# Snowdar/asv-subtools

Hardware: AMD Instinct MI355X
Metric: utterances/sec (200-frame) embedding extraction + EER, 1/2/4/8 MI355X (higher is better)
Workload: dtype bf16; 1 GPU; BASELINE configs[1]: standard TDNN x-vector: Xvector(80,10,training=False), 80-dim fbank, 256 utterances x 200 frames per GPU per step, features resident in HBM, f32 embeddings out; global_batch_utts=256, frames_per_utt=200, parallelism=utterance shards x1, streams=2

## Files before the change

### asv-subtools_amd/csrc/device_utils.h

```cpp
#pragma once
#include <hip/hip_runtime.h>
#include <stdint.h>

#include "asv_internal.h"

namespace asv {

typedef __attribute__((__vector_size__(8 * sizeof(__bf16)))) __bf16 bf16x8_t;
typedef __attribute__((__vector_size__(16 * sizeof(float)))) float f32x16_t;
typedef __attribute__((__vector_size__(4 * sizeof(float)))) float f32x4_t;

__host__ __device__ __forceinline__ int round_up_dev(int x, int m) { return (x + m - 1) / m * m; }

typedef _Float16 f16x8_t __attribute__((ext_vector_type(8)));
typedef _Float16 asv_f16x2 __attribute__((ext_vector_type(2)));

__device__ __forceinline__ float bf16_bits_to_f32(uint32_t h) { return __uint_as_float(h << 16); }

typedef float asv_f32x2 __attribute__((ext_vector_type(2)));
typedef __bf16 asv_bf16x2 __attribute__((ext_vector_type(2)));

__device__ __forceinline__ uint32_t pack_bf16x2(float lo, float hi) {
  const asv_f32x2 v = {lo, hi};
  return __builtin_bit_cast(uint32_t, __builtin_convertvector(v, asv_bf16x2));
}

__device__ __forceinline__ uint32_t f32_to_bf16_bits(float f) { return pack_bf16x2(f, 0.0f) & 0xffffu; }

template <int ET>
__device__ __forceinline__ uint32_t pack_h16x2(float lo, float hi) {
  static_assert(ET == ET_BF16 || ET == ET_F16, "16-bit element types only");
  const asv_f32x2 v = {lo, hi};
  if constexpr (ET == ET_BF16) return __builtin_bit_cast(uint32_t, __builtin_convertvector(v, asv_bf16x2));
  else return __builtin_bit_cast(uint32_t, __builtin_convertvector(v, asv_f16x2));
}
template <int ET>
__device__ __forceinline__ void unpack_h16x2(uint32_t w, float &lo, float &hi) {
  static_assert(ET == ET_BF16 || ET == ET_F16, "16-bit element types only");
  if constexpr (ET == ET_BF16) {
    lo = __uint_as_float(w << 16);
    hi = __uint_as_float(w & 0xffff0000u);
  } else {
    const asv_f32x2 f = __builtin_convertvector(__builtin_bit_cast(asv_f16x2, w), asv_f32x2);
    lo = f.x; hi = f.y;
  }
}
template <int ET>
__device__ __forceinline__ float h16_bits_to_f32(uint32_t h) {
  float lo, hi;
  unpack_h16x2<ET>(h, lo, hi);
  return lo;
}
template <int ET>
__device__ __forceinline__ uint32_t f32_to_h16_bits(float f) { return pack_h16x2<ET>(f, 0.0f) & 0xffffu; }

template <int ET>
__device__ __forceinline__ void unpack_h16x8(const uint4 u, float *v) {
  unpack_h16x2<ET>(u.x, v[0], v[1]); unpack_h16x2<ET>(u.y, v[2], v[3]);
  unpack_h16x2<ET>(u.z, v[4], v[5]); unpack_h16x2<ET>(u.w, v[6], v[7]);
}
template <int ET>
__device__ __forceinline__ uint4 pack_h16x8(const float *v) {
  return make_uint4(pack_h16x2<ET>(v[0], v[1]), pack_h16x2<ET>(v[2], v[3]), pack_h16x2<ET>(v[4], v[5]), pack_h16x2<ET>(v[6], v[7]));
}

template <int ET>
__device__ __forceinline__ f32x16_t mfma16(const uint4 a, const uint4 b, const f32x16_t c) {
  static_assert(ET == ET_BF16 || ET == ET_F16, "16-bit element types only");
  if constexpr (ET == ET_BF16) return __builtin_amdgcn_mfma_f32_32x32x16_bf16(__builtin_bit_cast(bf16x8_t, a), __builtin_bit_cast(bf16x8_t, b), c, 0, 0, 0);
  else return __builtin_amdgcn_mfma_f32_32x32x16_f16(__builtin_bit_cast(f16x8_t, a), __builtin_bit_cast(f16x8_t, b), c, 0, 0, 0);
}

__device__ __forceinline__ uint32_t relu_h16x2(uint32_t w) {
  typedef short s16x2 __attribute__((ext_vector_type(2)));
  const s16x2 z = {0, 0};
  return __builtin_bit_cast(uint32_t, __builtin_elementwise_max(__builtin_bit_cast(s16x2, w), z));
}

template <int ET>
__device__ __forceinline__ uint4 add_h16x8(uint4 a, uint4 b) {
  float va[8], vb[8];
  unpack_h16x8<ET>(a, va);
  unpack_h16x8<ET>(b, vb);
#pragma unroll
  for (int i = 0; i < 8; ++i) va[i] += vb[i];
  return pack_h16x8<ET>(va);
}
__device__ __forceinline__ uint4 add_bf16x8(uint4 a, uint4 b) { return add_h16x8<ET_BF16>(a, b); }

__device__ __forceinline__ uint4 add_f32x4(uint4 a, uint4 b) {
  uint4 r;
  r.x = __float_as_uint(__uint_as_float(a.x) + __uint_as_float(b.x));
  r.y = __float_as_uint(__uint_as_float(a.y) + __uint_as_float(b.y));
  r.z = __float_as_uint(__uint_as_float(a.z) + __uint_as_float(b.z));
  r.w = __float_as_uint(__uint_as_float(a.w) + __uint_as_float(b.w));
  return r;
}

struct X3Frag { uint4 hi, lo; };

__device__ __forceinline__ uint32_t h16_range_bits(uint32_t packed_hi) { return (packed_hi & 0x7fff7fffu) + 0x04000400u; }
__device__ __forceinline__ void x3_publish_range(uint32_t acc_bits, uint32_t *status) {
  if (status != nullptr && __builtin_amdgcn_ballot_w64((acc_bits & 0x80008000u) != 0u) != 0ull && (threadIdx.x & 63) == 0) atomicOr(status, ASV_STATUS_HALF_RANGE);
}

template <int ET, bool WITH_LO>
__device__ __forceinline__ X3Frag x3_split(const uint4 a, const uint4 b) {
  const float v[8] = {__uint_as_float(a.x), __uint_as_float(a.y), __uint_as_float(a.z), __uint_as_float(a.w),
                      __uint_as_float(b.x), __uint_as_float(b.y), __uint_as_float(b.z), __uint_as_float(b.w)};
  uint32_t h[4], l[4];
#pragma unroll
  for (int k = 0; k < 4; ++k) {
    h[k] = pack_h16x2<ET>(v[2 * k], v[2 * k + 1]);
    l[k] = 0u;
    if constexpr (WITH_LO) {
      float r0, r1;
      if constexpr (ET == ET_F16) {
        asm("v_fma_mix_f32 %0, %1, -1.0, %2 op_sel:[0,0,0] op_sel_hi:[1,0,0]" : "=v"(r0) : "v"(h[k]), "v"(v[2 * k]));
        asm("v_fma_mix_f32 %0, %1, -1.0, %2 op_sel:[1,0,0] op_sel_hi:[1,0,0]" : "=v"(r1) : "v"(h[k]), "v"(v[2 * k + 1]));
      } else {
        float h0, h1;
        unpack_h16x2<ET>(h[k], h0, h1);
        r0 = v[2 * k] - h0; r1 = v[2 * k + 1] - h1;
      }
      l[k] = pack_h16x2<ET>(r0, r1);
    }
  }
  X3Frag f;
  f.hi = make_uint4(h[0], h[1], h[2], h[3]);
  f.lo = make_uint4(l[0], l[1], l[2], l[3]);
  return f;
}
template <int ET, bool WITH_LO>
__device__ __forceinline__ X3Frag x3_split(const uint4 a, const uint4 b, uint32_t &range) {
  const X3Frag f = x3_split<ET, WITH_LO>(a, b);
  if constexpr (ET == ET_F16) range |= h16_range_bits(f.hi.x) | h16_range_bits(f.hi.y) | h16_range_bits(f.hi.z) | h16_range_bits(f.hi.w);
  return f;
}

constexpr int kScaleWhi = 127 + 6, kScaleWlo = 127 - 6, kScaleXlo = 127 - 11, kScaleXhi = 127;
typedef int v8i __attribute__((ext_vector_type(8)));

__device__ __forceinline__ uint32_t mx_range_bits(uint32_t packed_hi) { return (packed_hi & 0x7fff7fffu) + 0x05000500u; }

template <bool SEL>
__device__ __forceinline__ void split_mx(float v0, float v1, uint32_t &hi16, int &hi8, int &lo8, uint32_t &range) {
  hi16 = pack_h16x2<ET_F16>(v0, v1);
  range |= mx_range_bits(hi16);
  float r0, r1;
  asm("v_fma_mix_f32 %0, %1, -1.0, %2 op_sel:[0,0,0] op_sel_hi:[1,0,0]" : "=v"(r0) : "v"(hi16), "v"(v0));
  asm("v_fma_mix_f32 %0, %1, -1.0, %2 op_sel:[1,0,0] op_sel_hi:[1,0,0]" : "=v"(r1) : "v"(hi16), "v"(v1));
  hi8 = __builtin_amdgcn_cvt_pk_bf8_f32(v0, v1, hi8, SEL);
  lo8 = __builtin_amdgcn_cvt_pk_bf8_f32(r0 * 2048.0f, r1 * 2048.0f, lo8, SEL);
}

__device__ __forceinline__ double wave_sum_f64(double v) {
#pragma unroll
  for (int off = 32; off >= 1; off >>= 1) v += __shfl_xor(v, off);
  return v;
}

struct TrNo { static constexpr bool value = false; };
struct TrYes { static constexpr bool value = true; };

__device__ __forceinline__ float max_lo(float v, float lo) {
  float r;
  asm("v_max_f32 %0, %1, %2" : "=v"(r) : "v"(v), "v"(lo));
  return r;
}

__device__ __forceinline__ float apply_act(float v, int act) {
  switch (act) {
    case ASV_ACT_RELU: return fmaxf(v, 0.0f);
    case ASV_ACT_TANH: return tanhf(v);
    case ASV_ACT_SIGMOID: return 1.0f / (1.0f + expf(-v));
    default: return v;
  }
}

template <int ET>
__device__ __forceinline__ float load_elem(const void *base, size_t idx) {
  if constexpr (ET != ET_F32) return h16_bits_to_f32<ET>(reinterpret_cast<const uint16_t *>(base)[idx]);
  else return reinterpret_cast<const float *>(base)[idx];
}

template <int ET>
__device__ __forceinline__ void store_elem(void *base, size_t idx, float v) {
  if constexpr (ET != ET_F32) reinterpret_cast<uint16_t *>(base)[idx] = (uint16_t)f32_to_h16_bits<ET>(v);
  else reinterpret_cast<float *>(base)[idx] = v;
}

template <int RES_ET>
__device__ __forceinline__ float tdnn_epilogue(const TdnnKernelParams &p, float acc, int row, int ch,
                                               float bias, float scale, float shift, bool valid) {
  if (!valid) return 0.0f;
  float z = acc + bias;
  int seg = 0;
  if (p.seg_bias != nullptr || p.seg_scale != nullptr) seg = p.row_seg[row];
  if (p.seg_bias != nullptr) z += p.seg_bias[(size_t)seg * p.ld_segbias + ch];
  if (p.affine_first) {
    z = apply_act(z * scale + shift, p.act1);
  } else {
    z = apply_act(z, p.act1) * scale + shift;
  }
  z = apply_act(z, p.act2);
  if (p.seg_scale != nullptr) z *= p.seg_scale[(size_t)seg * p.ld_segscale + ch];
  if (p.res != nullptr) z += load_elem<RES_ET>(p.res, (size_t)row * p.ldres + ch);
  return z;
}

__device__ __forceinline__ float tdnn_epilogue_fast(float acc, float bias, float lo, float scale, float shift, bool valid) {
  const float z = fmaxf(acc + bias, lo) * scale + shift;
  return valid ? z : 0.0f;
}

__device__ __forceinline__ int xcd_swizzle(int bid, int nblocks) {
  const int xcd = bid & 7, q = nblocks >> 3, r = nblocks & 7;
  const int base = (xcd < r) ? xcd * (q + 1) : r * (q + 1) + (xcd - r) * q;
  return base + (bid >> 3);
}

}
```

### asv-subtools_amd/csrc/kernels_tdnn_chain.hip

```cpp
#include <cstdlib>

#include "chain_pool.h"
#include "lds_dma.h"

#ifndef CHAIN_EXP
#define CHAIN_EXP 0
#endif

namespace asv {
namespace {

constexpr int CN = kChainWidth;
constexpr int CBK = 64;
constexpr int CROWB = 128;
constexpr int CSTAGES = 4;
constexpr int YROWB = CN * 2;
template <int MF> struct ChainGeom {
  static constexpr int CM = MF * 32;
  static constexpr int CWIN = CM + 2 * kHalo;
  static constexpr int CSTAGE = CWIN * CROWB;
  static constexpr int CGROUPS = CWIN / 8;
  static constexpr int CPIECES = (CGROUPS + 7) / 8;
  static constexpr int Y_BYTES = CM * YROWB;
  static constexpr int SCR_OFF = Y_BYTES;
  static constexpr int LDS = Y_BYTES + 32768;
  static_assert(CSTAGES * CSTAGE <= Y_BYTES, "the window ring lives inside the Y region");
  static_assert(LDS <= 163840, "160 KiB of LDS per CU");
};

typedef float f32x2_t __attribute__((ext_vector_type(2)));

template <int POOLV, int ET = ET_BF16, int ABL = 0, int MF = 4>
__global__ __launch_bounds__(512, 2) void tdnn_chain_kernel(const TdnnChainParams p) {
  using Geo = ChainGeom<MF>;
  constexpr int CM = Geo::CM, CSTAGE = Geo::CSTAGE, CGROUPS = Geo::CGROUPS, CPIECES = Geo::CPIECES, SCR_OFF = Geo::SCR_OFF;
  __shared__ __attribute__((aligned(16))) unsigned char lds[Geo::LDS];
  const int tid = threadIdx.x, lane = tid & 63;
  const int wave = __builtin_amdgcn_readfirstlane(tid >> 6);
  const int lr = lane & 31, lh = lane >> 5;
  const int m0 = p.row_base + blockIdx.x * CM;
  const uint32_t lds_base = __builtin_amdgcn_readfirstlane((uint32_t)(uintptr_t)(lds_byte *)lds);
  float *par = reinterpret_cast<float *>(lds + SCR_OFF);

  int n_stamp = 0;
  auto stamp = [&]() {
    if (p.dbg != nullptr && lane == 0 && n_stamp < 14) p.dbg[((size_t)blockIdx.x * 8 + wave) * 32 + n_stamp] = __builtin_amdgcn_s_memtime();
    ++n_stamp;
  };
  auto fine = [&](int k) {
    if constexpr (ABL == 3) if (p.dbg != nullptr && lane == 0) p.dbg[((size_t)blockIdx.x * 8 + wave) * 32 + 16 + k] = __builtin_amdgcn_s_memtime();
  };
  stamp();
  if (p.dbg != nullptr && lane == 0) p.dbg[((size_t)blockIdx.x * 8 + wave) * 32 + 14] = __builtin_amdgcn_s_memrealtime();
  auto stage_params = [&](const TdnnChainLayer &L) {
    if (tid < 384) {
      const int which = tid >> 7, idx = (tid & 127) * 4;
      float4 v = (which == 1) ? make_float4(1.f, 1.f, 1.f, 1.f) : make_float4(0.f, 0.f, 0.f, 0.f);
      const float *src = (which == 0) ? L.bias : (which == 1 ? L.scale : L.shift);
      if (src != nullptr) v = *reinterpret_cast<const float4 *>(src + idx);
      *reinterpret_cast<float4 *>(par + which * CN + idx) = v;
    }
  };

  uint4 wf[4][2];
  f32x16_t acc[MF][2];
  struct XFrags { uint4 x[MF]; };
  auto init_acc = [&](const float *bias64) {
#pragma unroll
    for (int j = 0; j < 2; ++j)
#pragma unroll
      for (int q = 0; q < 4; ++q) {
        const float4 b4 = *reinterpret_cast<const float4 *>(bias64 + j * 32 + 8 * q + 4 * lh);
#pragma unroll
        for (int i = 0; i < MF; ++i) {
          acc[i][j][q * 4 + 0] = b4.x; acc[i][j][q * 4 + 1] = b4.y; acc[i][j][q * 4 + 2] = b4.z; acc[i][j][q * 4 + 3] = b4.w;
        }
      }
  };
  auto mma2 = [&](const XFrags &f, int kg, int j, int i0, auto tr) {
#pragma unroll
    for (int i = i0; i < i0 + 2 && i < MF; ++i) {
      if constexpr (decltype(tr)::value) acc[i][j] = mfma16<ET>(f.x[i], wf[kg][j], acc[i][j]);
      else acc[i][j] = mfma16<ET>(wf[kg][j], f.x[i], acc[i][j]);
    }
  };

  stage_params(p.first);
  {
    const unsigned char *xg = reinterpret_cast<const unsigned char *>(p.x);
    const size_t x_pitch = (size_t)p.ldx * 2;
    const int g_row = lane >> 3, g_slot = lane & 7;
    const int nchunks = p.cin_pad / CBK;
    const int n_taps = p.n_taps;
    uint32_t a_off[CPIECES];
#pragma unroll
    for (int i = 0; i < CPIECES; ++i) {
      const int grp = min(wave + i * 8, CGROUPS - 1);
      const int w = grp * 8 + g_row;
      const int row = min(max(m0 - kHalo + w, 0), p.rows - 1);
      a_off[i] = (uint32_t)row * (uint32_t)x_pitch + (uint32_t)lds_swz(w, g_slot) * 16u;
    }
    auto issue_A = [&](int c, int st) {
      const unsigned char *base = xg + (size_t)c * (CBK * 2);
#pragma unroll
      for (int i = 0; i < CPIECES; ++i) {
        const int grp = min(wave + i * 8, CGROUPS - 1);
        const uint32_t dst = __builtin_amdgcn_readfirstlane(lds_base + st * CSTAGE + grp * 1024);
        glds16_s(base, a_off[i], dst);
      }
    };
    const size_t frag_stride = (size_t)n_taps * nchunks * 4096;
    const unsigned char *wA0 = reinterpret_cast<const unsigned char *>(p.first.wfrag) + (size_t)(wave * 2) * frag_stride;
    const unsigned char *wA1 = wA0 + frag_stride;
    const uint32_t lane16 = (uint32_t)lane * 16u;
    auto x_base = [&](int c, int d) -> uint32_t {
      const int wrow = lr + kHalo + d;
      return (uint32_t)((c % CSTAGES) * CSTAGE + wrow * CROWB + ((lh ^ ((wrow >> 1) & 7)) << 4));
    };
    auto load_x4 = [&](uint32_t xb, int kg, int i, XFrags &f) {
      f.x[i] = *reinterpret_cast<const uint4 *>(lds + (xb ^ (uint32_t)(kg << 5)) + i * 4096);
    };
    issue_A(0, 0);
#pragma unroll
    for (int kg = 0; kg < 4; ++kg) {
      wf[kg][0] = *reinterpret_cast<const uint4 *>(wA0 + (size_t)kg * 1024 + lane16);
      wf[kg][1] = *reinterpret_cast<const uint4 *>(wA1 + (size_t)kg * 1024 + lane16);
    }
    if (nchunks > 2) {
      issue_A(1, 1);
      issue_A(2, 2);
      asm volatile("s_waitcnt vmcnt(%0)" ::"n"(2 * CPIECES) : "memory");
    } else {
      if (nchunks > 1) issue_A(1, 1);
      asm volatile("s_waitcnt vmcnt(0)" ::: "memory");
    }
    __builtin_amdgcn_s_barrier();
    asm volatile("" ::: "memory");
    stamp();
    init_acc(p.first.bias + wave * 64);
    const int v_taps = p.taps[lane < 9 ? lane : 0];
    const int d_first = __builtin_amdgcn_readlane(v_taps, 0);
    XFrags x0, x1;
    uint32_t xb = x_base(0, d_first);
#pragma unroll
    for (int i = 0; i < MF; ++i) load_x4(xb, 0, i, x0);
#pragma unroll 1
    for (int c = 0; c < nchunks; ++c) {
      for (int t = 0; t < n_taps; ++t) {
        const bool last_tap = (t + 1 == n_taps);
        int cn = c, tn = t + 1;
        if (last_tap) { tn = 0; cn = c + 1; }
        const bool more = cn < nchunks;
        if (!more) { cn = c; tn = t; }
        const size_t wnext = ((size_t)tn * nchunks + cn) * 4096;
        auto group = [&](const XFrags &xc, int kg, XFrags &xn, uint32_t xbn, int kgn) {
#pragma unroll
          for (int q = 0; q < 4; ++q) {
            if (q < MF) load_x4(xbn, kgn, q, xn);
            mma2(xc, kg, q / 2, (q % 2) * 2, TrNo{});
            if (q == 1) wf[kg][0] = *reinterpret_cast<const uint4 *>(wA0 + wnext + (size_t)kg * 1024 + lane16);
            if (q == 3) wf[kg][1] = *reinterpret_cast<const uint4 *>(wA1 + wnext + (size_t)kg * 1024 + lane16);
            __builtin_amdgcn_sched_barrier(0);
          }
        };
        group(x0, 0, x1, xb, 1);
        group(x1, 1, x0, xb, 2);
        group(x0, 2, x1, xb, 3);
        if (last_tap && c + 1 < nchunks) {
          asm volatile("s_waitcnt vmcnt(8)" ::: "memory");
          __builtin_amdgcn_s_barrier();
          asm volatile("" ::: "memory");
          if (c + 3 < nchunks) issue_A(c + 3, (c + 3) % CSTAGES);
        }
        const uint32_t xbn = x_base(cn, __builtin_amdgcn_readlane(v_taps, tn));
        group(x1, 3, x0, xbn, 0);
        xb = xbn;
      }
    }
  }

  auto store_Y = [&](int relu, bool affine) {
    const float act_lo = relu ? 0.0f : -INFINITY;
    unsigned char *yrow = lds + lr * YROWB + lh * 8;
    const int rx = lr & 15;
    if (!affine) {
#pragma unroll
      for (int j = 0; j < 2; ++j)
#pragma unroll
        for (int q = 0; q < 4; ++q) {
          unsigned char *dst = yrow + (((wave * 8 + j * 4 + q) ^ rx) << 4);
#pragma unroll
          for (int i = 0; i < MF; ++i) {
            uint2 pk;
            pk.x = pack_h16x2<ET>(acc[i][j][q * 4 + 0], acc[i][j][q * 4 + 1]);
            pk.y = pack_h16x2<ET>(acc[i][j][q * 4 + 2], acc[i][j][q * 4 + 3]);
            if (relu) { pk.x = relu_h16x2(pk.x); pk.y = relu_h16x2(pk.y); }
            *reinterpret_cast<uint2 *>(dst + i * 32 * YROWB) = pk;
          }
        }
      return;
    }
#pragma unroll
    for (int j = 0; j < 2; ++j)
#pragma unroll
      for (int q = 0; q < 4; ++q) {
        const int chl = wave * 64 + j * 32 + 8 * q + 4 * lh;
        const float4 sc4 = *reinterpret_cast<const float4 *>(par + CN + chl);
        const float4 sh4 = *reinterpret_cast<const float4 *>(par + 2 * CN + chl);
        const float sc[4] = {sc4.x, sc4.y, sc4.z, sc4.w}, sh[4] = {sh4.x, sh4.y, sh4.z, sh4.w};
        unsigned char *dst = yrow + (((wave * 8 + j * 4 + q) ^ rx) << 4);
#pragma unroll
        for (int i = 0; i < MF; ++i) {
          float y[4];
#pragma unroll
          for (int e = 0; e < 4; ++e) y[e] = fmaf(max_lo(acc[i][j][q * 4 + e], act_lo), sc[e], sh[e]);
          uint2 pk;
          pk.x = pack_h16x2<ET>(y[0], y[1]);
          pk.y = pack_h16x2<ET>(y[2], y[3]);
          *reinterpret_cast<uint2 *>(dst + i * 32 * YROWB) = pk;
        }
      }
  };

  auto yloop = [&](const unsigned char *wb0, const unsigned char *wb1, const float *bias64, auto tr) {
    const uint32_t lane16 = (uint32_t)lane * 16u;
    const uint32_t yb = (uint32_t)(lr * YROWB);
    const uint32_t sx = (uint32_t)(lh ^ (lr & 15));
    auto load_y4 = [&](int c, int kg, int i, XFrags &f) {
      f.x[i] = *reinterpret_cast<const uint4 *>(lds + yb + ((((uint32_t)(c * 8 + kg * 2)) ^ sx) << 4) + i * 32 * YROWB);
    };
#pragma unroll
    for (int kg = 0; kg < 4; ++kg) {
      wf[kg][0] = *reinterpret_cast<const uint4 *>(wb0 + (size_t)kg * 1024 + lane16);
      wf[kg][1] = *reinterpret_cast<const uint4 *>(wb1 + (size_t)kg * 1024 + lane16);
    }
    if constexpr (decltype(tr)::value) {
      const float b0 = bias64[lr], b1 = bias64[32 + lr];
#pragma unroll
      for (int i = 0; i < MF; ++i)
#pragma unroll
        for (int r = 0; r < 16; ++r) { acc[i][0][r] = b0; acc[i][1][r] = b1; }
    } else {
      init_acc(bias64);
    }
    XFrags x0, x1;
#pragma unroll
    for (int i = 0; i < MF; ++i) load_y4(0, 0, i, x0);
#pragma unroll 1
    for (int c = 0; c < CN / CBK; ++c) {
      const int cn = min(c + 1, CN / CBK - 1);
      const size_t wnext = (CHAIN_EXP & 4) ? 0 : (size_t)cn * 4096;
      auto group = [&](const XFrags &xc, int kg, XFrags &xn, int c2, int kgn) {
#pragma unroll
        for (int q = 0; q < 4; ++q) {
          if (q < MF) load_y4(c2, kgn, q, xn);
          mma2(xc, kg, q / 2, (q % 2) * 2, tr);
          if (q == 1 && !(CHAIN_EXP & 2)) wf[kg][0] = *reinterpret_cast<const uint4 *>(wb0 + wnext + (size_t)kg * 1024 + lane16);
          if (q == 3 && !(CHAIN_EXP & 1)) wf[kg][1] = *reinterpret_cast<const uint4 *>(wb1 + wnext + (size_t)kg * 1024 + lane16);
          __builtin_amdgcn_sched_barrier(0);
        }
      };
      group(x0, 0, x1, c, 1);
      group(x1, 1, x0, c, 2);
      group(x0, 2, x1, c, 3);
      group(x1, 3, x0, cn, 0);
    }
  };

  stamp();
  asm volatile("s_waitcnt vmcnt(0)" ::: "memory");
  __builtin_amdgcn_s_barrier();
  asm volatile("" ::: "memory");
  stamp();
  store_Y(p.first.relu, p.first.scale != nullptr);
  __builtin_amdgcn_s_barrier();
  asm volatile("" ::: "memory");
  stamp();

#pragma unroll 1
  for (int m = 0; m < p.n_mid; ++m) {
    const TdnnChainLayer &L = p.mid[m];
    stage_params(L);
    const size_t frag_stride = (size_t)(CN / CBK) * 4096;
    const unsigned char *wb = reinterpret_cast<const unsigned char *>(L.wfrag) + (size_t)(wave * 2) * frag_stride;
    yloop(wb, wb + frag_stride, L.bias + wave * 64, TrNo{});
    stamp();
    asm volatile("s_waitcnt vmcnt(0) lgkmcnt(0)" ::: "memory");
    __builtin_amdgcn_s_barrier();
    asm volatile("" ::: "memory");
    store_Y(L.relu, L.scale != nullptr);
    __builtin_amdgcn_s_barrier();
    asm volatile("" ::: "memory");
    stamp();
  }

  {
    const TdnnChainLayer &L = p.last;
    const float act_lo = L.relu ? 0.0f : -INFINITY;
    const int half = p.tile_base + (int)blockIdx.x;
    const int first_seg = pool_first_seg(p, m0);
    const int rowseg_lo = (m0 + lane < p.rows) ? p.row_seg[m0 + lane] : -1;
    const int rowseg_hi = (64 + lane < CM && m0 + 64 + lane < p.rows) ? p.row_seg[m0 + 64 + lane] : -1;
    const size_t frag_stride = (size_t)(CN / CBK) * 4096;
#pragma unroll 1
    for (int cb = wave * 64; cb < L.cout_pad; cb += 512) {
      const unsigned char *wb = reinterpret_cast<const unsigned char *>(L.wfrag) + (size_t)(cb / 32) * frag_stride;
      yloop(wb, wb + frag_stride, L.bias + cb, TrYes{});
      if constexpr (ABL == 4) __builtin_amdgcn_s_barrier();
      stamp();
      if constexpr (ABL == 1) {
#if defined(__HIP_DEVICE_COMPILE__)
#pragma unroll
        for (int i = 0; i < MF; ++i) asm volatile("" ::"v"(acc[i][0]), "v"(acc[i][1]));
#endif
        stamp();
        continue;
      }
      const float sc[2] = {(ABL != 2 && L.scale != nullptr) ? L.scale[cb + lr] : 1.0f, (ABL != 2 && L.scale != nullptr) ? L.scale[cb + 32 + lr] : 1.0f};
      if constexpr (POOLV == 0) {
        float ps[2] = {0.f, 0.f}, pq[2] = {0.f, 0.f}, pv[2] = {0.f, 0.f};
        int cur_seg = -1;
        auto publish = [&](bool mine) {
          if (mine) pool_publish_moments(p, half, first_seg, cur_seg, cb, lr, lh, ps, pq, pv, sc);
        };
  #pragma unroll
        for (int i = 0; i < MF; ++i) {
          const int rs_vec = (i < 2) ? rowseg_lo : rowseg_hi;
          const unsigned long long in_frag = 0xffffffffull << ((i & 1) * 32);
          const unsigned long long m_valid = __builtin_amdgcn_ballot_w64(rs_vec >= 0) & in_frag;
          if (m_valid == 0) continue;
          const int sg0 = __builtin_amdgcn_readlane(rs_vec, __builtin_ctzll(m_valid));
          const unsigned long long m_same = __builtin_amdgcn_ballot_w64(rs_vec == sg0) & in_frag;
          if (m_same == in_frag) {
            const bool chg = cur_seg != sg0;
            if (__builtin_amdgcn_ballot_w64(chg) != 0) {
              publish(chg);
  #pragma unroll
              for (int j = 0; j < 2; ++j) {
                const float v0 = max_lo(acc[i][j][0], act_lo);
                ps[j] = chg ? 0.0f : ps[j]; pq[j] = chg ? 0.0f : pq[j]; pv[j] = chg ? v0 : pv[j];
              }
              cur_seg = chg ? sg0 : cur_seg;
            }
  #pragma unroll
            for (int j = 0; j < 2; ++j) {
              float s4[4] = {0.f, 0.f, 0.f, 0.f}, q4[4] = {0.f, 0.f, 0.f, 0.f};
  #pragma unroll
              for (int r = 0; r < 16; ++r) {
                const float dlt = max_lo(acc[i][j][r], act_lo) - pv[j];
                s4[r & 3] += dlt;
                q4[r & 3] = fmaf(dlt, dlt, q4[r & 3]);
              }
              ps[j] += (s4[0] + s4[1]) + (s4[2] + s4[3]);
              pq[j] += (q4[0] + q4[1]) + (q4[2] + q4[3]);
            }
          } else {
  #pragma unroll
            for (int r = 0; r < 16; ++r) {
              const int f = (i & 1) * 32 + 8 * (r >> 2) + (r & 3);
              const int sg_a = __builtin_amdgcn_readlane(rs_vec, f), sg_b = __builtin_amdgcn_readlane(rs_vec, f + 4);
              const int sg = lh ? sg_b : sg_a;
              const bool ok = sg >= 0;
              const bool chg = ok && sg != cur_seg;
              if (__builtin_amdgcn_ballot_w64(chg) != 0) {
                publish(chg);
  #pragma unroll
                for (int j = 0; j < 2; ++j) {
                  const float v0 = max_lo(acc[i][j][r], act_lo);
                  ps[j] = chg ? 0.0f : ps[j]; pq[j] = chg ? 0.0f : pq[j]; pv[j] = chg ? v0 : pv[j];
                }
                cur_seg = chg ? sg : cur_seg;
              }
  #pragma unroll
              for (int j = 0; j < 2; ++j) {
                const float dlt = ok ? max_lo(acc[i][j][r], act_lo) - pv[j] : 0.0f;
                ps[j] += dlt;
                pq[j] = fmaf(dlt, dlt, pq[j]);
              }
            }
          }
        }
        publish(true);
      } else {
        float ps[2] = {0.f, 0.f}, pq[2] = {0.f, 0.f}, pv[2] = {0.f, 0.f};
        const bool first_unit = ABL == 3 && cb < 512;
        if (first_unit) fine(0);
        int cur_seg = -1;
        bool have = false;
        auto publish = [&]() {
          if constexpr (ABL == 2) { asm volatile("" ::"v"(ps[0]), "v"(ps[1]), "v"(pq[0]), "v"(pq[1]), "v"(pv[0]), "v"(pv[1])); return; }
          pool_publish_moments(p, half, first_seg, cur_seg, cb, lr, lh, ps, pq, pv, sc);
        };
  #pragma unroll
        for (int i = 0; i < MF; ++i) {
          const int rs_vec = (i < 2) ? rowseg_lo : rowseg_hi;
          const int shift = (i & 1) * 32;
          uint32_t rem = (uint32_t)(__builtin_amdgcn_ballot_w64(rs_vec >= 0) >> shift);
          if (rem == 0) continue;
          float u[2][16];
  #pragma unroll
          for (int j = 0; j < 2; ++j)
  #pragma unroll
            for (int r = 0; r < 16; ++r) u[j][r] = max_lo(acc[i][j][r], act_lo);
          while (rem != 0) {
            const int sg = __builtin_amdgcn_readlane(rs_vec, shift + __builtin_ctz(rem));
            const uint32_t bits = (uint32_t)(__builtin_amdgcn_ballot_w64(rs_vec == sg) >> shift) & rem;
            rem &= ~bits;
            const bool fresh = sg != cur_seg;
            if (fresh) {
              publish();
              cur_seg = sg;
              have = false;
  #pragma unroll
              for (int j = 0; j < 2; ++j) { ps[j] = 0.0f; pq[j] = 0.0f; }
            }
            if (bits == 0xffffffffu) {
              const bool need = !have;
              have = true;
  #pragma unroll
              for (int j = 0; j < 2; ++j) {
                pv[j] = need ? u[j][0] : pv[j];
                const f32x2_t pv2 = {pv[j], pv[j]};
                f32x2_t s2[2] = {{0.f, 0.f}, {0.f, 0.f}}, q2[2] = {{0.f, 0.f}, {0.f, 0.f}};
  #pragma unroll
                for (int r = 0; r < 16; r += 2) {
                  const f32x2_t uu = {u[j][r], u[j][r + 1]};
                  const f32x2_t d = uu - pv2;
                  s2[(r >> 1) & 1] += d;
                  q2[(r >> 1) & 1] = __builtin_elementwise_fma(d, d, q2[(r >> 1) & 1]);
                }
                const f32x2_t st = s2[0] + s2[1], qt = q2[0] + q2[1];
                ps[j] += st.x + st.y;
                pq[j] += qt.x + qt.y;
              }
            } else {
              const uint32_t x = bits >> (4 * lh);
              const uint32_t lm = (x & 0xfu) | ((x >> 4) & 0xf0u) | ((x >> 8) & 0xf00u) | ((x >> 12) & 0xf000u);
              const bool need = !have && lm != 0;
              if (__builtin_amdgcn_ballot_w64(need) != 0) {
                const int rsel = need ? __builtin_ctz(lm) : 16;
  #pragma unroll
                for (int r = 15; r >= 0; --r) {
                  const bool hit = rsel == r;
                  pv[0] = hit ? u[0][r] : pv[0];
                  pv[1] = hit ? u[1][r] : pv[1];
                }
                have = have || need;
              }
              f32x2_t s2[2] = {{0.f, 0.f}, {0.f, 0.f}}, q2[2] = {{0.f, 0.f}, {0.f, 0.f}};
              const f32x2_t pva = {pv[0], pv[0]}, pvb = {pv[1], pv[1]};
  #pragma unroll
              for (int r = 0; r < 16; r += 2) {
                const int t0 = (int)(lm << (31 - r)) >> 31, t1 = (int)(lm << (30 - r)) >> 31;
                f32x2_t da = (f32x2_t){u[0][r], u[0][r + 1]} - pva, db = (f32x2_t){u[1][r], u[1][r + 1]} - pvb;
                da.x = __int_as_float(__float_as_int(da.x) & t0); da.y = __int_as_float(__float_as_int(da.y) & t1);
                db.x = __int_as_float(__float_as_int(db.x) & t0); db.y = __int_as_float(__float_as_int(db.y) & t1);
                s2[0] += da; q2[0] = __builtin_elementwise_fma(da, da, q2[0]);
                s2[1] += db; q2[1] = __builtin_elementwise_fma(db, db, q2[1]);
              }
              ps[0] += s2[0].x + s2[0].y; pq[0] += q2[0].x + q2[0].y;
              ps[1] += s2[1].x + s2[1].y; pq[1] += q2[1].x + q2[1].y;
            }
          }
          if (first_unit) fine(1 + i);
        }
        publish();
        if (first_unit) fine(5);
      }
      if constexpr (ABL == 4) __builtin_amdgcn_s_barrier();
      stamp();
    }
    if (p.dbg != nullptr && lane == 0) p.dbg[((size_t)blockIdx.x * 8 + wave) * 32 + 15] = __builtin_amdgcn_s_memrealtime();
  }
}

}

ChainTilePlan chain_tile_plan(int rows, bool allow_tail) {
  ChainTilePlan plan;
  const int n = rows / 128;
  plan.n128 = n;
  static const int mode = getenv("ASV_AMD_CHAIN_TAIL") != nullptr ? atoi(getenv("ASV_AMD_CHAIN_TAIL")) : 1;
  if (!allow_tail || mode == 0) return plan;
  int dev = 0, cus = 256;
  if (hipGetDevice(&dev) == hipSuccess) (void)hipDeviceGetAttribute(&cus, hipDeviceAttributeMultiprocessorCount, dev);
  if (n < cus) {
    for (int r : {64, 96}) {
      const int t = (rows + r - 1) / r;
      if (t <= cus) { plan.n128 = 0; plan.n_tail = t; plan.tail_rows = r; return plan; }
    }
    return plan;
  }
  if (mode == 2) {
    const int tail = n % cus, as96 = (tail * 128 + 95) / 96;
    if (tail > 0 && as96 <= cus) { plan.n128 = n - tail; plan.n_tail = as96; plan.tail_rows = 96; }
  }
  return plan;
}

int launch_tdnn_chain(const TdnnChainParams &p0, hipStream_t s) {
  TdnnChainParams p = p0;
  constexpr int CM = 128;
  ASV_REQUIRE(p.rows % CM == 0 && p.rows >= CM, "tdnn(chain): rows %d not a multiple of %d", p.rows, CM);
  ASV_REQUIRE(p.cin_pad % CBK == 0 && p.cin_pad >= CBK && p.n_taps >= 1 && p.n_taps <= ASV_MAX_TAPS, "tdnn(chain): first layer with %d channels / %d taps", p.cin_pad, p.n_taps);
  ASV_REQUIRE((unsigned long long)p.rows * (unsigned long long)p.ldx * 2ull < (1ull << 32), "tdnn(chain): input matrix beyond 32-bit offsets");
  ASV_REQUIRE(p.first.wfrag && p.last.wfrag && p.last.bias && p.n_mid >= 0 && p.n_mid <= 2 && p.last.cout_pad % 64 == 0, "tdnn(chain): incomplete layer description");
  ASV_REQUIRE(p.pool_partial && p.row_seg && p.pool_slots >= 1, "tdnn(chain): the last layer feeds the fused pooling (partials / row map missing)");
  for (int t = 0; t < p.n_taps; ++t) ASV_REQUIRE(p.taps[t] >= -kHalo && p.taps[t] <= kHalo, "tdnn(chain): tap offset %d exceeds the %d-frame halo", p.taps[t], kHalo);
  if (p.n128 == 0 && p.n_tail == 0) p.n128 = p.rows / CM;
  ASV_REQUIRE(p.n_tail == 0 || p.tail_rows == 96 || p.tail_rows == 64, "tdnn(chain): tail tiles of %d frames", p.tail_rows);
  ASV_REQUIRE(p.n128 * 128 + p.n_tail * p.tail_rows >= p.rows && p.n128 * 128 <= p.rows, "tdnn(chain): tile plan %d x 128 + %d x %d does not cover %d rows", p.n128, p.n_tail,
              p.tail_rows, p.rows);
  const dim3 block(512);
  p.row_base = 0; p.tile_base = 0;
#ifdef ASV_WITH_ABLATION
  static const bool live = getenv("ASV_AMD_LIVE_TUNE") != nullptr;
  auto read_int = [](const char *name) { const char *v = getenv(name); return v != nullptr ? atoi(v) : -1; };
  static const int poolv0 = read_int("ASV_AMD_CHAIN_POOLV"), abl0 = read_int("ASV_AMD_CHAIN_ABL");
  const int poolv = live ? read_int("ASV_AMD_CHAIN_POOLV") : poolv0, abl = live ? read_int("ASV_AMD_CHAIN_ABL") : abl0;
  static const int waves0 = read_int("ASV_AMD_CHAIN_WAVES");
  const int waves = live ? read_int("ASV_AMD_CHAIN_WAVES") : waves0;
  if (p.n_tail == 0) {
    const dim3 grid(p.n128);
    if (waves == 4 && abl <= 0 && poolv != 0 && !(p.dbg != nullptr && p.dbg_fine) && tdnn_chain4_supported(p)) return launch_tdnn_chain4(p, s);
    if (p.et == ET_BF16 && !(p.dbg != nullptr && p.dbg_fine) && (abl == 1 || abl == 2 || (abl == 4 && p.last.cout_pad % 512 == 0) || poolv == 0)) {
      if (abl == 1) hipLaunchKernelGGL((tdnn_chain_kernel<1, ET_BF16, 1>), grid, block, 0, s, p);
      else if (abl == 2) hipLaunchKernelGGL((tdnn_chain_kernel<1, ET_BF16, 2>), grid, block, 0, s, p);
      else if (abl == 4) hipLaunchKernelGGL((tdnn_chain_kernel<1, ET_BF16, 4>), grid, block, 0, s, p);
      else hipLaunchKernelGGL(tdnn_chain_kernel<0>, grid, block, 0, s, p);
      ASV_HIP_CHECK(hipGetLastError());
      return ASV_OK;
    }
  }
#endif
  if (p.n128 > 0) {
    const dim3 grid(p.n128);
    if (p.et == ET_F16) hipLaunchKernelGGL((tdnn_chain_kernel<1, ET_F16>), grid, block, 0, s, p);
    else if (p.dbg != nullptr && p.dbg_fine) hipLaunchKernelGGL((tdnn_chain_kernel<1, ET_BF16, 3>), grid, block, 0, s, p);
    else hipLaunchKernelGGL(tdnn_chain_kernel<1>, grid, block, 0, s, p);
  }
  if (p.n_tail > 0) {
    p.row_base = p.n128 * 128; p.tile_base = p.n128;
    p.dbg = nullptr;
    const dim3 grid(p.n_tail);
    if (p.tail_rows == 96) {
      if (p.et == ET_F16) hipLaunchKernelGGL((tdnn_chain_kernel<1, ET_F16, 0, 3>), grid, block, 0, s, p);
      else hipLaunchKernelGGL((tdnn_chain_kernel<1, ET_BF16, 0, 3>), grid, block, 0, s, p);
    } else {
      if (p.et == ET_F16) hipLaunchKernelGGL((tdnn_chain_kernel<1, ET_F16, 0, 2>), grid, block, 0, s, p);
      else hipLaunchKernelGGL((tdnn_chain_kernel<1, ET_BF16, 0, 2>), grid, block, 0, s, p);
    }
  }
  ASV_HIP_CHECK(hipGetLastError());
  return ASV_OK;
}

}
```

Measured before the change: 950,400 utterances/s.

## Use 16x16x32 MFMA shape for first and middle TDNN chain layers

Adds a 16x16x32 MFMA helper and alternate code paths in the fused TDNN chain kernel, covering the first-layer window loop, the middle-layer Y loops, the store epilogue and, optionally, the last layer's pooling epilogue. By default (CHAIN_MFMA_SHAPES=1) the first and middle layers use the narrow MFMA shape, while the last layer keeps the 32x32 path. The goal is better MFMA throughput or scheduling from the smaller instruction shape. The cost is twice as many accumulator fragments, new LDS and weight fragment addressing, and possible extra register pressure under 512-thread launch bounds.

Measured after the change: 985,100 utterances/s (median of 6 runs). +3.7%, better.

```diff
diff --git a/asv-subtools_amd/csrc/device_utils.h b/asv-subtools_amd/csrc/device_utils.h
--- a/asv-subtools_amd/csrc/device_utils.h
+++ b/asv-subtools_amd/csrc/device_utils.h
@@ -69,6 +69,13 @@
   static_assert(ET == ET_BF16 || ET == ET_F16, "16-bit element types only");
   if constexpr (ET == ET_BF16) return __builtin_amdgcn_mfma_f32_32x32x16_bf16(__builtin_bit_cast(bf16x8_t, a), __builtin_bit_cast(bf16x8_t, b), c, 0, 0, 0);
   else return __builtin_amdgcn_mfma_f32_32x32x16_f16(__builtin_bit_cast(f16x8_t, a), __builtin_bit_cast(f16x8_t, b), c, 0, 0, 0);
+}
+
+template <int ET>
+__device__ __forceinline__ f32x4_t mfma16n(const uint4 a, const uint4 b, const f32x4_t c) {
+  static_assert(ET == ET_BF16 || ET == ET_F16, "16-bit element types only");
+  if constexpr (ET == ET_BF16) return __builtin_amdgcn_mfma_f32_16x16x32_bf16(__builtin_bit_cast(bf16x8_t, a), __builtin_bit_cast(bf16x8_t, b), c, 0, 0, 0);
+  else return __builtin_amdgcn_mfma_f32_16x16x32_f16(__builtin_bit_cast(f16x8_t, a), __builtin_bit_cast(f16x8_t, b), c, 0, 0, 0);
 }
 
 __device__ __forceinline__ uint32_t relu_h16x2(uint32_t w) {
diff --git a/asv-subtools_amd/csrc/kernels_tdnn_chain.hip b/asv-subtools_amd/csrc/kernels_tdnn_chain.hip
--- a/asv-subtools_amd/csrc/kernels_tdnn_chain.hip
+++ b/asv-subtools_amd/csrc/kernels_tdnn_chain.hip
@@ -30,14 +30,16 @@
 
 typedef float f32x2_t __attribute__((ext_vector_type(2)));
 
-template <int POOLV, int ET = ET_BF16, int ABL = 0, int MF = 4>
+template <int POOLV, int ET = ET_BF16, int ABL = 0, int MF = 4, int NY = 0, int NL = 0>
 __global__ __launch_bounds__(512, 2) void tdnn_chain_kernel(const TdnnChainParams p) {
   using Geo = ChainGeom<MF>;
+  static_assert(!NL || (POOLV == 1 && (ABL == 0 || ABL == 3)), "the narrow last layer has the run-based pooling epilogue only");
   constexpr int CM = Geo::CM, CSTAGE = Geo::CSTAGE, CGROUPS = Geo::CGROUPS, CPIECES = Geo::CPIECES, SCR_OFF = Geo::SCR_OFF;
   __shared__ __attribute__((aligned(16))) unsigned char lds[Geo::LDS];
   const int tid = threadIdx.x, lane = tid & 63;
   const int wave = __builtin_amdgcn_readfirstlane(tid >> 6);
   const int lr = lane & 31, lh = lane >> 5;
+  const int lc = lane & 15, lo = lane >> 4;
   const int m0 = p.row_base + blockIdx.x * CM;
   const uint32_t lds_base = __builtin_amdgcn_readfirstlane((uint32_t)(uintptr_t)(lds_byte *)lds);
   float *par = reinterpret_cast<float *>(lds + SCR_OFF);
@@ -82,6 +84,29 @@
     for (int i = i0; i < i0 + 2 && i < MF; ++i) {
       if constexpr (decltype(tr)::value) acc[i][j] = mfma16<ET>(f.x[i], wf[kg][j], acc[i][j]);
       else acc[i][j] = mfma16<ET>(wf[kg][j], f.x[i], acc[i][j]);
+    }
+  };
+
+  uint4 wn[2][4];
+  f32x4_t accn[2 * MF][4];
+  struct XFragsN { uint4 x[2 * MF]; };
+  const uint32_t lane16n = (uint32_t)((lo >> 1) * 1024 + ((lo & 1) * 32 + lc) * 16);
+  auto load_wn = [&](const unsigned char *w0, const unsigned char *w1, size_t at, int kg2, int cf) {
+    wn[kg2][cf] = *reinterpret_cast<const uint4 *>(((cf >> 1) ? w1 : w0) + at + (size_t)(kg2 * 2048 + (cf & 1) * 256) + lane16n);
+  };
+  auto init_acc_n = [&](const float *bias64) {
+#pragma unroll
+    for (int cf = 0; cf < 4; ++cf) {
+      const float4 b4 = *reinterpret_cast<const float4 *>(bias64 + 16 * cf + 4 * lo);
+#pragma unroll
+      for (int f = 0; f < 2 * MF; ++f) { accn[f][cf][0] = b4.x; accn[f][cf][1] = b4.y; accn[f][cf][2] = b4.z; accn[f][cf][3] = b4.w; }
+    }
+  };
+  auto mma_n = [&](const XFragsN &f, int kg2, int s, auto tr) {
+#pragma unroll
+    for (int i = (s & 1) * MF; i < (s & 1) * MF + MF; ++i) {
+      if constexpr (decltype(tr)::value) accn[i][s >> 1] = mfma16n<ET>(f.x[i], wn[kg2][s >> 1], accn[i][s >> 1]);
+      else accn[i][s >> 1] = mfma16n<ET>(wn[kg2][s >> 1], f.x[i], accn[i][s >> 1]);
     }
   };
 
@@ -120,11 +145,25 @@
     auto load_x4 = [&](uint32_t xb, int kg, int i, XFrags &f) {
       f.x[i] = *reinterpret_cast<const uint4 *>(lds + (xb ^ (uint32_t)(kg << 5)) + i * 4096);
     };
+    auto x_base_n = [&](int c, int d) -> uint32_t {
+      const int wrow = lc + kHalo + d;
+      return (uint32_t)((c % CSTAGES) * CSTAGE + wrow * CROWB + ((lo ^ ((wrow >> 1) & 7)) << 4));
+    };
+    auto load_xn = [&](uint32_t xb, int kg2, int f, XFragsN &fr) {
+      fr.x[f] = *reinterpret_cast<const uint4 *>(lds + (xb ^ (uint32_t)(kg2 << 6)) + f * 2048);
+    };
     issue_A(0, 0);
-#pragma unroll
-    for (int kg = 0; kg < 4; ++kg) {
-      wf[kg][0] = *reinterpret_cast<const uint4 *>(wA0 + (size_t)kg * 1024 + lane16);
-      wf[kg][1] = *reinterpret_cast<const uint4 *>(wA1 + (size_t)kg * 1024 + lane16);
+    if constexpr (NY) {
+#pragma unroll
+      for (int kg2 = 0; kg2 < 2; ++kg2)
+#pragma unroll
+        for (int cf = 0; cf < 4; ++cf) load_wn(wA0, wA1, 0, kg2, cf);
+    } else {
+#pragma unroll
+      for (int kg = 0; kg < 4; ++kg) {
+        wf[kg][0] = *reinterpret_cast<const uint4 *>(wA0 + (size_t)kg * 1024 + lane16);
+        wf[kg][1] = *reinterpret_cast<const uint4 *>(wA1 + (size_t)kg * 1024 + lane16);
+      }
     }
     if (nchunks > 2) {
       issue_A(1, 1);
@@ -137,9 +176,46 @@
     __builtin_amdgcn_s_barrier();
     asm volatile("" ::: "memory");
     stamp();
-    init_acc(p.first.bias + wave * 64);
     const int v_taps = p.taps[lane < 9 ? lane : 0];
     const int d_first = __builtin_amdgcn_readlane(v_taps, 0);
+    if constexpr (NY) {
+      init_acc_n(p.first.bias + wave * 64);
+      XFragsN y0, y1;
+      uint32_t xb = x_base_n(0, d_first);
+#pragma unroll
+      for (int f = 0; f < 2 * MF; ++f) load_xn(xb, 0, f, y0);
+#pragma unroll 1
+      for (int c = 0; c < nchunks; ++c) {
+        for (int t = 0; t < n_taps; ++t) {
+          const bool last_tap = (t + 1 == n_taps);
+          int cn = c, tn = t + 1;
+          if (last_tap) { tn = 0; cn = c + 1; }
+          const bool more = cn < nchunks;
+          if (!more) { cn = c; tn = t; }
+          const size_t wnext = ((size_t)tn * nchunks + cn) * 4096;
+          auto group = [&](const XFragsN &xc, int kg2, XFragsN &xn, uint32_t xbn, int kg2n) {
+#pragma unroll
+            for (int s = 0; s < 8; ++s) {
+              if (s < 2 * MF) load_xn(xbn, kg2n, s, xn);
+              mma_n(xc, kg2, s, TrNo{});
+              if (s & 1) load_wn(wA0, wA1, wnext, kg2, s >> 1);
+              __builtin_amdgcn_sched_barrier(0);
+            }
+          };
+          group(y0, 0, y1, xb, 1);
+          if (last_tap && c + 1 < nchunks) {
+            asm volatile("s_waitcnt vmcnt(%0)" ::"n"(4 + CPIECES) : "memory");
+            __builtin_amdgcn_s_barrier();
+            asm volatile("" ::: "memory");
+            if (c + 3 < nchunks) issue_A(c + 3, (c + 3) % CSTAGES);
+          }
+          const uint32_t xbn = x_base_n(cn, __builtin_amdgcn_readlane(v_taps, tn));
+          group(y1, 1, y0, xbn, 0);
+          xb = xbn;
+        }
+      }
+    } else {
+    init_acc(p.first.bias + wave * 64);
     XFrags x0, x1;
     uint32_t xb = x_base(0, d_first);
 #pragma unroll
@@ -177,6 +253,7 @@
         xb = xbn;
       }
     }
+    }
   }
 
   auto store_Y = [&](int relu, bool affine) {
@@ -222,6 +299,84 @@
       }
   };
 
+  auto store_Y_n = [&](int relu, bool affine) {
+    const float act_lo = relu ? 0.0f : -INFINITY;
+    unsigned char *yrow = lds + lc * YROWB + (lo & 1) * 8;
+    auto body = [&](auto aff) {
+    constexpr bool affine = decltype(aff)::value;
+#pragma unroll
+    for (int cf = 0; cf < 4; ++cf) {
+      unsigned char *dst = yrow + (((wave * 8 + cf * 2 + (lo >> 1)) ^ lc) << 4);
+      float sc[4] = {1.f, 1.f, 1.f, 1.f}, sh[4] = {0.f, 0.f, 0.f, 0.f};
+      if constexpr (affine) {
+        const int chl = wave * 64 + 16 * cf + 4 * lo;
+        const float4 sc4 = *reinterpret_cast<const float4 *>(par + CN + chl);
+        const float4 sh4 = *reinterpret_cast<const float4 *>(par + 2 * CN + chl);
+        sc[0] = sc4.x; sc[1] = sc4.y; sc[2] = sc4.z; sc[3] = sc4.w;
+        sh[0] = sh4.x; sh[1] = sh4.y; sh[2] = sh4.z; sh[3] = sh4.w;
+      }
+#pragma unroll
+      for (int f = 0; f < 2 * MF; ++f) {
+        uint2 pk;
+        if constexpr (affine) {
+          float y[4];
+#pragma unroll
+          for (int e = 0; e < 4; ++e) y[e] = fmaf(max_lo(accn[f][cf][e], act_lo), sc[e], sh[e]);
+          pk.x = pack_h16x2<ET>(y[0], y[1]);
+          pk.y = pack_h16x2<ET>(y[2], y[3]);
+        } else {
+          pk.x = pack_h16x2<ET>(accn[f][cf][0], accn[f][cf][1]);
+          pk.y = pack_h16x2<ET>(accn[f][cf][2], accn[f][cf][3]);
+          if (relu) { pk.x = relu_h16x2(pk.x); pk.y = relu_h16x2(pk.y); }
+        }
+        *reinterpret_cast<uint2 *>(dst + f * 16 * YROWB) = pk;
+      }
+    }
+    };
+    if (affine) body(TrYes{}); else body(TrNo{});
+  };
+
+  auto yloop_n = [&](const unsigned char *wb0, const unsigned char *wb1, const float *bias64, auto tr) {
+    const uint32_t yb = (uint32_t)(lc * YROWB);
+    const uint32_t sx = (uint32_t)(lo ^ lc);
+    auto load_yn = [&](int c, int kg2, int f, XFragsN &fr) {
+      fr.x[f] = *reinterpret_cast<const uint4 *>(lds + yb + ((((uint32_t)(c * 8 + kg2 * 4)) ^ sx) << 4) + f * 16 * YROWB);
+    };
+#pragma unroll
+    for (int kg2 = 0; kg2 < 2; ++kg2)
+#pragma unroll
+      for (int cf = 0; cf < 4; ++cf) load_wn(wb0, wb1, 0, kg2, cf);
+    if constexpr (decltype(tr)::value) {
+#pragma unroll
+      for (int cf = 0; cf < 4; ++cf) {
+        const float b = bias64[16 * cf + lc];
+#pragma unroll
+        for (int f = 0; f < 2 * MF; ++f) { accn[f][cf][0] = b; accn[f][cf][1] = b; accn[f][cf][2] = b; accn[f][cf][3] = b; }
+      }
+    } else {
+      init_acc_n(bias64);
+    }
+    XFragsN y0, y1;
+#pragma unroll
+    for (int f = 0; f < 2 * MF; ++f) load_yn(0, 0, f, y0);
+#pragma unroll 1
+    for (int c = 0; c < CN / CBK; ++c) {
+      const int cn = min(c + 1, CN / CBK - 1);
+      const size_t wnext = (size_t)cn * 4096;
+      auto group = [&](const XFragsN &xc, int kg2, XFragsN &xn, int c2, int kg2n) {
+#pragma unroll
+        for (int s = 0; s < 8; ++s) {
+          if (s < 2 * MF) load_yn(c2, kg2n, s, xn);
+          mma_n(xc, kg2, s, tr);
+          if (s & 1) load_wn(wb0, wb1, wnext, kg2, s >> 1);
+          __builtin_amdgcn_sched_barrier(0);
+        }
+      };
+      group(y0, 0, y1, c, 1);
+      group(y1, 1, y0, cn, 0);
+    }
+  };
+
   auto yloop = [&](const unsigned char *wb0, const unsigned char *wb1, const float *bias64, auto tr) {
     const uint32_t lane16 = (uint32_t)lane * 16u;
     const uint32_t yb = (uint32_t)(lr * YROWB);
@@ -272,7 +427,7 @@
   __builtin_amdgcn_s_barrier();
   asm volatile("" ::: "memory");
   stamp();
-  store_Y(p.first.relu, p.first.scale != nullptr);
+  if constexpr (NY) store_Y_n(p.first.relu, p.first.scale != nullptr); else store_Y(p.first.relu, p.first.scale != nullptr);
   __builtin_amdgcn_s_barrier();
   asm volatile("" ::: "memory");
   stamp();
@@ -283,12 +438,12 @@
     stage_params(L);
     const size_t frag_stride = (size_t)(CN / CBK) * 4096;
     const unsigned char *wb = reinterpret_cast<const unsigned char *>(L.wfrag) + (size_t)(wave * 2) * frag_stride;
-    yloop(wb, wb + frag_stride, L.bias + wave * 64, TrNo{});
+    if constexpr (NY) yloop_n(wb, wb + frag_stride, L.bias + wave * 64, TrNo{}); else yloop(wb, wb + frag_stride, L.bias + wave * 64, TrNo{});
     stamp();
     asm volatile("s_waitcnt vmcnt(0) lgkmcnt(0)" ::: "memory");
     __builtin_amdgcn_s_barrier();
     asm volatile("" ::: "memory");
-    store_Y(L.relu, L.scale != nullptr);
+    if constexpr (NY) store_Y_n(L.relu, L.scale != nullptr); else store_Y(L.relu, L.scale != nullptr);
     __builtin_amdgcn_s_barrier();
     asm volatile("" ::: "memory");
     stamp();
@@ -305,7 +460,7 @@
 #pragma unroll 1
     for (int cb = wave * 64; cb < L.cout_pad; cb += 512) {
       const unsigned char *wb = reinterpret_cast<const unsigned char *>(L.wfrag) + (size_t)(cb / 32) * frag_stride;
-      yloop(wb, wb + frag_stride, L.bias + cb, TrYes{});
+      if constexpr (NL) yloop_n(wb, wb + frag_stride, L.bias + cb, TrYes{}); else yloop(wb, wb + frag_stride, L.bias + cb, TrYes{});
       if constexpr (ABL == 4) __builtin_amdgcn_s_barrier();
       stamp();
       if constexpr (ABL == 1) {
@@ -317,7 +472,94 @@
         continue;
       }
       const float sc[2] = {(ABL != 2 && L.scale != nullptr) ? L.scale[cb + lr] : 1.0f, (ABL != 2 && L.scale != nullptr) ? L.scale[cb + 32 + lr] : 1.0f};
-      if constexpr (POOLV == 0) {
+      if constexpr (NL) {
+        float ps[4] = {0.f, 0.f, 0.f, 0.f}, pq[4] = {0.f, 0.f, 0.f, 0.f}, pv[4] = {0.f, 0.f, 0.f, 0.f};
+        float scn[4];
+#pragma unroll
+        for (int cf = 0; cf < 4; ++cf) scn[cf] = L.scale != nullptr ? L.scale[cb + 16 * cf + lc] : 1.0f;
+        const bool first_unit = ABL == 3 && cb < 512;
+        if (first_unit) fine(0);
+        int cur_seg = -1;
+        bool have = false;
+        auto publish = [&]() {
+          if (cur_seg < 0) return;
+          float ts[4], tq[4];
+#pragma unroll
+          for (int cf = 0; cf < 4; ++cf) { ts[cf] = ps[cf] + __shfl_xor(ps[cf], 32); tq[cf] = pq[cf] + __shfl_xor(pq[cf], 32); }
+          if (lo < 2) {
+#pragma unroll
+            for (int h = 0; h < 2; ++h) {
+              const float a[2] = {ts[h], ts[2 + h]}, b[2] = {tq[h], tq[2 + h]}, c[2] = {pv[h], pv[2 + h]}, d[2] = {scn[h], scn[2 + h]};
+              pool_publish_moments(p, half, first_seg, cur_seg, cb, 16 * h + lc, lo, a, b, c, d);
+            }
+          }
+        };
+#pragma unroll
+        for (int f = 0; f < 2 * MF; ++f) {
+          const int rs_vec = (f < 4) ? rowseg_lo : rowseg_hi;
+          const int shift = (f & 3) * 16;
+          uint32_t rem = (uint32_t)(__builtin_amdgcn_ballot_w64(rs_vec >= 0) >> shift) & 0xffffu;
+          if (rem != 0) {
+            float u[4][4];
+#pragma unroll
+            for (int cf = 0; cf < 4; ++cf)
+#pragma unroll
+              for (int e = 0; e < 4; ++e) u[cf][e] = max_lo(accn[f][cf][e], act_lo);
+            while (rem != 0) {
+              const int sg = __builtin_amdgcn_readlane(rs_vec, shift + __builtin_ctz(rem));
+              const uint32_t bits = (uint32_t)(__builtin_amdgcn_ballot_w64(rs_vec == sg) >> shift) & rem;
+              rem &= ~bits;
+              if (sg != cur_seg) {
+                publish();
+                cur_seg = sg;
+                have = false;
+#pragma unroll
+                for (int cf = 0; cf < 4; ++cf) { ps[cf] = 0.0f; pq[cf] = 0.0f; }
+              }
+              const uint32_t lm = (bits >> (4 * lo)) & 0xfu, lmp = (bits >> (4 * (lo ^ 2))) & 0xfu;
+              const bool need = !have && (lm | lmp) != 0;
+              if (__builtin_amdgcn_ballot_w64(need) != 0) {
+                const int rsel = lm != 0 ? __builtin_ctz(lm) : 0;
+                const bool own = (lo < 2) ? lm != 0 : lmp == 0;
+#pragma unroll
+                for (int cf = 0; cf < 4; ++cf) {
+                  float c = u[cf][0];
+#pragma unroll
+                  for (int e = 1; e < 4; ++e) c = (rsel == e) ? u[cf][e] : c;
+                  const float o = __shfl_xor(c, 32);
+                  pv[cf] = need ? (own ? c : o) : pv[cf];
+                }
+                have = have || need;
+              }
+              if (bits == 0xffffu) {
+#pragma unroll
+                for (int cf = 0; cf < 4; ++cf) {
+                  const f32x2_t pv2 = {pv[cf], pv[cf]};
+                  const f32x2_t d0 = (f32x2_t){u[cf][0], u[cf][1]} - pv2, d1 = (f32x2_t){u[cf][2], u[cf][3]} - pv2;
+                  const f32x2_t st = d0 + d1, qt = __builtin_elementwise_fma(d1, d1, d0 * d0);
+                  ps[cf] += st.x + st.y;
+                  pq[cf] += qt.x + qt.y;
+                }
+              } else {
+                const int t0 = (int)(lm << 31) >> 31, t1 = (int)(lm << 30) >> 31, t2 = (int)(lm << 29) >> 31, t3 = (int)(lm << 28) >> 31;
+#pragma unroll
+                for (int cf = 0; cf < 4; ++cf) {
+                  const f32x2_t pv2 = {pv[cf], pv[cf]};
+                  f32x2_t d0 = (f32x2_t){u[cf][0], u[cf][1]} - pv2, d1 = (f32x2_t){u[cf][2], u[cf][3]} - pv2;
+                  d0.x = __int_as_float(__float_as_int(d0.x) & t0); d0.y = __int_as_float(__float_as_int(d0.y) & t1);
+                  d1.x = __int_as_float(__float_as_int(d1.x) & t2); d1.y = __int_as_float(__float_as_int(d1.y) & t3);
+                  const f32x2_t st = d0 + d1, qt = __builtin_elementwise_fma(d1, d1, d0 * d0);
+                  ps[cf] += st.x + st.y;
+                  pq[cf] += qt.x + qt.y;
+                }
+              }
+            }
+          }
+          if (first_unit && (f & 1)) fine(1 + f / 2);
+        }
+        publish();
+        if (first_unit) fine(5);
+      } else if constexpr (POOLV == 0) {
         float ps[2] = {0.f, 0.f}, pq[2] = {0.f, 0.f}, pv[2] = {0.f, 0.f};
         int cur_seg = -1;
         auto publish = [&](bool mine) {
@@ -496,6 +738,34 @@
     if (tail > 0 && as96 <= cus) { plan.n128 = n - tail; plan.n_tail = as96; plan.tail_rows = 96; }
   }
   return plan;
+}
+
+#ifndef CHAIN_MFMA_SHAPES
+#define CHAIN_MFMA_SHAPES 1
+#endif
+constexpr int kChainNarrowY = CHAIN_MFMA_SHAPES & 1, kChainNarrowL = (CHAIN_MFMA_SHAPES >> 1) & 1;
+
+template <int NY, int NL>
+static void launch_chain_forms(TdnnChainParams p, hipStream_t s) {
+  const dim3 block(512);
+  if (p.n128 > 0) {
+    const dim3 grid(p.n128);
+    if (p.et == ET_F16) hipLaunchKernelGGL((tdnn_chain_kernel<1, ET_F16, 0, 4, NY, NL>), grid, block, 0, s, p);
+    else if (p.dbg != nullptr && p.dbg_fine) hipLaunchKernelGGL((tdnn_chain_kernel<1, ET_BF16, 3, 4, NY, NL>), grid, block, 0, s, p);
+    else hipLaunchKernelGGL((tdnn_chain_kernel<1, ET_BF16, 0, 4, NY, NL>), grid, block, 0, s, p);
+  }
+  if (p.n_tail > 0) {
+    p.row_base = p.n128 * 128; p.tile_base = p.n128;
+    p.dbg = nullptr;
+    const dim3 grid(p.n_tail);
+    if (p.tail_rows == 96) {
+      if (p.et == ET_F16) hipLaunchKernelGGL((tdnn_chain_kernel<1, ET_F16, 0, 3, NY, NL>), grid, block, 0, s, p);
+      else hipLaunchKernelGGL((tdnn_chain_kernel<1, ET_BF16, 0, 3, NY, NL>), grid, block, 0, s, p);
+    } else {
+      if (p.et == ET_F16) hipLaunchKernelGGL((tdnn_chain_kernel<1, ET_F16, 0, 2, NY, NL>), grid, block, 0, s, p);
+      else hipLaunchKernelGGL((tdnn_chain_kernel<1, ET_BF16, 0, 2, NY, NL>), grid, block, 0, s, p);
+    }
+  }
 }
 
 int launch_tdnn_chain(const TdnnChainParams &p0, hipStream_t s) {
@@ -511,15 +781,18 @@
   ASV_REQUIRE(p.n_tail == 0 || p.tail_rows == 96 || p.tail_rows == 64, "tdnn(chain): tail tiles of %d frames", p.tail_rows);
   ASV_REQUIRE(p.n128 * 128 + p.n_tail * p.tail_rows >= p.rows && p.n128 * 128 <= p.rows, "tdnn(chain): tile plan %d x 128 + %d x %d does not cover %d rows", p.n128, p.n_tail,
               p.tail_rows, p.rows);
-  const dim3 block(512);
   p.row_base = 0; p.tile_base = 0;
 #ifdef ASV_WITH_ABLATION
+  const dim3 block(512);
+  int mfma = -1;
   static const bool live = getenv("ASV_AMD_LIVE_TUNE") != nullptr;
   auto read_int = [](const char *name) { const char *v = getenv(name); return v != nullptr ? atoi(v) : -1; };
   static const int poolv0 = read_int("ASV_AMD_CHAIN_POOLV"), abl0 = read_int("ASV_AMD_CHAIN_ABL");
   const int poolv = live ? read_int("ASV_AMD_CHAIN_POOLV") : poolv0, abl = live ? read_int("ASV_AMD_CHAIN_ABL") : abl0;
   static const int waves0 = read_int("ASV_AMD_CHAIN_WAVES");
   const int waves = live ? read_int("ASV_AMD_CHAIN_WAVES") : waves0;
+  static const int mfma0 = read_int("ASV_AMD_CHAIN_MFMA");
+  mfma = live ? read_int("ASV_AMD_CHAIN_MFMA") : mfma0;
   if (p.n_tail == 0) {
     const dim3 grid(p.n128);
     if (waves == 4 && abl <= 0 && poolv != 0 && !(p.dbg != nullptr && p.dbg_fine) && tdnn_chain4_supported(p)) return launch_tdnn_chain4(p, s);
@@ -533,24 +806,14 @@
     }
   }
 #endif
-  if (p.n128 > 0) {
-    const dim3 grid(p.n128);
-    if (p.et == ET_F16) hipLaunchKernelGGL((tdnn_chain_kernel<1, ET_F16>), grid, block, 0, s, p);
-    else if (p.dbg != nullptr && p.dbg_fine) hipLaunchKernelGGL((tdnn_chain_kernel<1, ET_BF16, 3>), grid, block, 0, s, p);
-    else hipLaunchKernelGGL(tdnn_chain_kernel<1>, grid, block, 0, s, p);
-  }
-  if (p.n_tail > 0) {
-    p.row_base = p.n128 * 128; p.tile_base = p.n128;
-    p.dbg = nullptr;
-    const dim3 grid(p.n_tail);
-    if (p.tail_rows == 96) {
-      if (p.et == ET_F16) hipLaunchKernelGGL((tdnn_chain_kernel<1, ET_F16, 0, 3>), grid, block, 0, s, p);
-      else hipLaunchKernelGGL((tdnn_chain_kernel<1, ET_BF16, 0, 3>), grid, block, 0, s, p);
-    } else {
-      if (p.et == ET_F16) hipLaunchKernelGGL((tdnn_chain_kernel<1, ET_F16, 0, 2>), grid, block, 0, s, p);
-      else hipLaunchKernelGGL((tdnn_chain_kernel<1, ET_BF16, 0, 2>), grid, block, 0, s, p);
-    }
-  }
+#ifdef ASV_WITH_ABLATION
+  if (mfma == 0) launch_chain_forms<0, 0>(p, s);
+  else if (mfma == 1) launch_chain_forms<1, 0>(p, s);
+  else if (mfma == 2) launch_chain_forms<0, 1>(p, s);
+  else if (mfma == 3) launch_chain_forms<1, 1>(p, s);
+  else
+#endif
+  launch_chain_forms<kChainNarrowY, kChainNarrowL>(p, s);
   ASV_HIP_CHECK(hipGetLastError());
   return ASV_OK;
 }
```
